# facebookresearch/ProcedureVRL

Measured on AMD Instinct MI355X. Metric: training clips/sec (8f x 224^2, ViT-B TimeSformer), higher is better.
Workload: dtype f16; 1 GPU; TimeSformer ViT-B 8x224^2, 32 clips/GPU, K=9871 step logits, top-5 KL + all-gather InfoNCE, fwd+bwd+AdamW (BASELINE configs[1]; configs[2] at 8 GPUs); clips_per_gpu=32, global_batch=32, parallelism=dp1

## Files before the change

include/pvrl.h:

```cpp
#ifndef PVRL_H_
#define PVRL_H_
#include <stdint.h>
#ifdef __cplusplus
extern "C" {
#endif

#define PVRL_EPI_BF16 0
#define PVRL_EPI_GELU 1
#define PVRL_EPI_QGELU 2
#define PVRL_EPI_RESID_F32 3
#define PVRL_EPI_F32 4
#define PVRL_EPI_DGELU 5
#define PVRL_EPI_DQGELU 6
#define PVRL_EPI_RESID_16 7
#define PVRL_EPI_GELU_ONLY 8

int pvrl_operand_dtype(void);

#define PVRL_NT_SKINNY_MAX_M 192
#define PVRL_NT_SKINNY_K 256
int pvrl_gemm_nt_bf16(const void* A, int64_t lda, const void* W, int64_t ldw, int64_t M, int64_t N, int64_t K,
                      int epilogue, const float* bias, const float* rowscale, const void* aux, int64_t aux_ld,
                      int64_t aux_rowmod, void* out0, int64_t ld0, void* out1, int64_t ld1, const float* bias2,
                      void* stream);

typedef struct pvrl_nt_problem {
  const void* A; int64_t lda;
  const void* W; int64_t ldw;
  int64_t M, N, K;
  const float* bias;
  const float* rowscale;
  const void* aux; int64_t aux_ld;
  void* out0; int64_t ld0;
} pvrl_nt_problem;
int pvrl_gemm_nt_batched_bf16(int nprob, const pvrl_nt_problem* problems, int epilogue, void* stream);

int64_t pvrl_gemm_nt_f32_small_workspace_bytes(int64_t M, int64_t N, int64_t K);
int pvrl_gemm_nt_f32_small(const float* A, int64_t lda, const float* B, int64_t ldb, const float* bias, float alpha,
                           float* C, int64_t ldc, int64_t M, int64_t N, int64_t K, void* workspace,
                           int64_t workspace_bytes, void* stream);

int64_t pvrl_gemm_tn_plan_splits(int64_t M, int64_t N, int64_t K);
int64_t pvrl_gemm_tn_workspace_bytes(int64_t N, int64_t K, int64_t splits);
int pvrl_gemm_tn_bf16(const void* P, int64_t ldp, const void* Q, int64_t ldq, int64_t M, int64_t N, int64_t K,
                      int64_t splits, float beta, float* dW, float* dbias, void* workspace, int64_t workspace_bytes,
                      const float* gscale, float* nonfinite, void* stream);
int pvrl_gemm_tn_into_bf16(const void* P, int64_t ldp, const void* Q, int64_t ldq, int64_t M, int64_t N, int64_t K,
                           int64_t splits, float beta, float* dW, int64_t ldw, int64_t n_valid, int64_t k_valid,
// ... 268 lines not shown
```

procedurevrl_amd/csrc/common.h:

```cpp
#pragma once
#include <hip/hip_runtime.h>
#include <stdint.h>
#include <stdlib.h>

#if defined(PVRL_OPERAND_F16)
typedef _Float16 op_t;
#define PVRL_OPERAND_CODE 1
#define MFMA_16x16x32 __builtin_amdgcn_mfma_f32_16x16x32_f16
#define MFMA_32x32x16 __builtin_amdgcn_mfma_f32_32x32x16_f16
#define FDOT2_F32 __builtin_amdgcn_fdot2
#else
typedef __bf16 op_t;
#define PVRL_OPERAND_CODE 0
#define MFMA_16x16x32 __builtin_amdgcn_mfma_f32_16x16x32_bf16
#define MFMA_32x32x16 __builtin_amdgcn_mfma_f32_32x32x16_bf16
#define FDOT2_F32 __builtin_amdgcn_fdot2_f32_bf16
#endif
typedef op_t opx2 __attribute__((ext_vector_type(2)));
typedef op_t opx4 __attribute__((ext_vector_type(4)));
typedef op_t opx8 __attribute__((ext_vector_type(8)));
typedef short s16x4 __attribute__((ext_vector_type(4)));
typedef float f32x2 __attribute__((ext_vector_type(2)));
typedef float f32x4 __attribute__((ext_vector_type(4)));
typedef float f32x16 __attribute__((ext_vector_type(16)));
// ... 51 lines not shown
#pragma unroll
  for (int o = 32; o > 0; o >>= 1) v = fmaxf(v, __shfl_xor(v, o, 64));
  return v;
}

__device__ __forceinline__ float gelu_clamp6(float u) {
  const float a = fabsf(u);
  return a > 6.0f ? 6.0f : a;
}
__device__ __forceinline__ float gelu_erf(float u) {
  const float x = gelu_clamp6(u);
  float p = fmaf(-2.9932052711956203e-05f, x, 0.0007281892467290163f);
  p = fmaf(p, x, -0.007909782230854034f);
  p = fmaf(p, x, 0.053108397871255875f);
  p = fmaf(p, x, 0.45901164412498474f);
  p = fmaf(p, x, 1.1511247158050537f);
  p = fmaf(p, x, 1.0f);
  const float h = __builtin_amdgcn_exp2f(-p);
  return fmaf(-x, h, fmaxf(u, 0.0f));
}
typedef float f32x2_t __attribute__((ext_vector_type(2)));
__device__ __forceinline__ f32x2_t gelu_erf2(f32x2_t u) {
  const f32x2_t x = {gelu_clamp6(u[0]), gelu_clamp6(u[1])};
  f32x2_t p = __builtin_elementwise_fma((f32x2_t)(-2.9932052711956203e-05f), x, (f32x2_t)(0.0007281892467290163f));
  p = __builtin_elementwise_fma(p, x, (f32x2_t)(-0.007909782230854034f));
  p = __builtin_elementwise_fma(p, x, (f32x2_t)(0.053108397871255875f));
  p = __builtin_elementwise_fma(p, x, (f32x2_t)(0.45901164412498474f));
  p = __builtin_elementwise_fma(p, x, (f32x2_t)(1.1511247158050537f));
  p = __builtin_elementwise_fma(p, x, (f32x2_t)(1.0f));
  const f32x2_t h = {__builtin_amdgcn_exp2f(-p[0]), __builtin_amdgcn_exp2f(-p[1])};
  const f32x2_t r = {fmaxf(u[0], 0.0f), fmaxf(u[1], 0.0f)};
  return __builtin_elementwise_fma(-x, h, r);
}
__device__ __forceinline__ float gelu_erf_grad(float u) {
  const float x = gelu_clamp6(u);
  const float e = __builtin_amdgcn_exp2f(x * x * -0.72134752044448170368f);
  float n = fmaf(1.678248281677952e-06f, x, -3.60403792001307e-05f);
  n = fmaf(n, x, 0.00034598674392327666f);
  n = fmaf(n, x, -0.002000307897105813f);
  n = fmaf(n, x, 0.008002669550478458f);
  n = fmaf(n, x, -0.024410134181380272f);
  n = fmaf(n, x, 0.061244383454322815f);
  n = fmaf(n, x, -0.13256259262561798f);
  n = fmaf(n, x, 0.24993102252483368f);
  n = fmaf(n, x, -0.7978806495666504f);
  n = fmaf(n, x, 0.5f);
  return 0.5f + copysignf(0.5f - e * n, u);
}
__device__ __forceinline__ float quick_gelu(float u) {
  return u * __builtin_amdgcn_rcpf(1.0f + __expf(-1.702f * u));
}
__device__ __forceinline__ float quick_gelu_grad(float u) {
  const float s = __builtin_amdgcn_rcpf(1.0f + __expf(-1.702f * u));
  return s * (1.0f + 1.702f * u * (1.0f - s));
}

__device__ __forceinline__ int xcd_remap(int bid, int nwg) {
  const int q = nwg >> 3, r = nwg & 7;
  const int xcd = bid & 7, idx = bid >> 3;
  const int base = (xcd < r) ? xcd * (q + 1) : r * (q + 1) + (xcd - r) * q;
  return base + idx;
}

static inline int cdiv(long a, long b) { return (int)((a + b - 1) / b); }

static inline int pvrl_compute_cus_per_xcd() {
// ... 13 lines not shown
```

procedurevrl_amd/csrc/gemm_nt.hip:

```cpp
#include "gemm_nt_core.h"
#include "gemm_nt8_core.h"
#include "gemm_nt_skinny.h"

bool pvrl_cls_gemm_f32(const float* A, int64_t lda, const float* B, int64_t ldb, const float* bias, float alpha, float* C, int64_t ldc,
                       int64_t M, int64_t N, int64_t K, hipStream_t s, int* status);

namespace {

constexpr int SG_T = 64, SG_K = 32, SG_LD = 68;
__global__ __launch_bounds__(256) void gemm_f32_small_kernel(const float* __restrict__ A, long lda,
                                                             const float* __restrict__ B, long ldb,
                                                             const float* __restrict__ bias, float alpha,
                                                             float* __restrict__ C, long ldc, int M, int N, int K,
                                                             int kchunk, float* __restrict__ part) {
  __shared__ __attribute__((aligned(16))) float sa[SG_K][SG_LD];
  __shared__ __attribute__((aligned(16))) float sb[SG_K][SG_LD];
  const int tid = threadIdx.x;
  const int n0 = blockIdx.x * SG_T, m0 = blockIdx.y * SG_T;
  const int kbeg = blockIdx.z * kchunk, kend = min(K, kbeg + kchunk);
  const int tx = tid & 15, ty = tid >> 4;
  const int lrow = tid >> 2, lk = (tid & 3) * 8;
  float acc[4][4];
#pragma unroll
  for (int i = 0; i < 4; ++i)
// ... 44 lines not shown
  }
}

__global__ __launch_bounds__(256) void f32_small_reduce_kernel(const float* __restrict__ part, int splits, long MN, int N,
                                                               const float* __restrict__ bias, float alpha,
                                                               float* __restrict__ C, long ldc) {
  for (long i = (long)blockIdx.x * 256 + threadIdx.x; i < MN; i += (long)gridDim.x * 256) {
    float a = 0.f;
    for (int z = 0; z < splits; ++z) a += part[(long)z * MN + i];
    const long m = i / N;
    const int n = (int)(i - m * N);
    C[m * ldc + n] = alpha * a + (bias ? bias[n] : 0.f);
  }
}

static int f32_small_plan(int64_t M, int64_t N, int64_t K, int* kchunk_out) {
  const int tiles = cdiv(N, SG_T) * cdiv(M, SG_T);
  int splits = 1;
  if (tiles < 128 && K >= 512) {
    splits = 256 / tiles;
    const int maxs = (int)(K / 128);
    if (splits > maxs) splits = maxs;
    if (splits < 1) splits = 1;
  }
  const int kchunk = cdiv(cdiv(K, splits), SG_K) * SG_K;
  if (kchunk_out) *kchunk_out = kchunk;
  return cdiv(K, kchunk);
}

constexpr int NT_MID_M = 2048;

template <int EPI>
int launch_nt(const GemmNT& p, hipStream_t s) {
  constexpr bool act_out = EPI == PVRL_EPI_GELU || EPI == PVRL_EPI_QGELU || EPI == PVRL_EPI_GELU_ONLY;
  if (nt_skinny_ok(p)) return launch_nt_skinny<EPI>(p, s);
  if (p.N == 768 && p.M >= 4096 && p.M < 20000) return launch_tile<EPI, 2, 6>(p, s);
  if (p.M >= 4096 && p.N % 256 == 0) {
    if (p.K >= 2 * BK && !(EPI == PVRL_EPI_RESID_16 && p.aux_rowmod != 0)) return launch_nt8<EPI>(p, s);
    return launch_tile<EPI, 4, 4>(p, s);
  }
  if (p.M >= 4096 && p.N % 256 != 0) {
    if (p.N % 384 == 0 && p.M >= 100000) return launch_tile<EPI, 2, 6>(p, s);
    if (p.N % 320 == 0) return launch_tile<EPI, 2, 5>(p, s);
  }
  if (p.M >= NT_MID_M && (p.N % 256 == 0 || act_out)) return launch_tile<EPI, 4, 2>(p, s);
  return launch_tile<EPI, 2, 2>(p, s);
}

}

extern "C" int pvrl_gemm_nt_bf16(const void* A, int64_t lda, const void* W, int64_t ldw, int64_t M, int64_t N,
                                 int64_t K, int epilogue, const float* bias, const float* rowscale,
                                 const void* aux, int64_t aux_ld, int64_t aux_rowmod, void* out0, int64_t ld0,
                                 void* out1, int64_t ld1, const float* bias2, void* stream) {
  if (M <= 0) return PVRL_OK;
  if (bias2 && epilogue != PVRL_EPI_RESID_F32 && epilogue != PVRL_EPI_RESID_16) return PVRL_EINVAL;
  if (!A || !W || !out0 || N <= 0 || K <= 0 || (N % 128) || (K % BK)) return PVRL_EINVAL;
  if ((lda % 8) || (ldw % 8) || (ld0 % 8)) return PVRL_EINVAL;
  if ((epilogue == PVRL_EPI_GELU || epilogue == PVRL_EPI_QGELU) && (!out1 || (ld1 % 8))) return PVRL_EINVAL;
  if ((epilogue == PVRL_EPI_RESID_F32 || epilogue == PVRL_EPI_RESID_16 || epilogue == PVRL_EPI_DGELU || epilogue == PVRL_EPI_DQGELU) &&
      (!aux || (aux_ld % 8)))
    return PVRL_EINVAL;
  GemmNT p;
  p.A = (const op_t*)A; p.lda = lda; p.W = (const op_t*)W; p.ldw = ldw;
  p.M = (int)M; p.N = (int)N; p.K = (int)K;
  p.bias = bias; p.bias2 = bias2; p.rowscale = rowscale; p.aux = aux; p.aux_ld = aux_ld; p.aux_rowmod = (int)aux_rowmod;
  p.out0 = out0; p.ld0 = ld0; p.out1 = out1; p.ld1 = ld1; p.m_off = 0; p.gm = 0;
  p.cus = pvrl_compute_cus_per_xcd(); p.tails = 1;
  hipStream_t s = (hipStream_t)stream;
  switch (epilogue) {
    case PVRL_EPI_BF16: return launch_nt<PVRL_EPI_BF16>(p, s);
    case PVRL_EPI_GELU: return launch_nt<PVRL_EPI_GELU>(p, s);
    case PVRL_EPI_QGELU: return launch_nt<PVRL_EPI_QGELU>(p, s);
    case PVRL_EPI_RESID_F32: return launch_nt<PVRL_EPI_RESID_F32>(p, s);
    case PVRL_EPI_F32: return launch_nt<PVRL_EPI_F32>(p, s);
    case PVRL_EPI_DGELU: return launch_nt<PVRL_EPI_DGELU>(p, s);
    case PVRL_EPI_DQGELU: return launch_nt<PVRL_EPI_DQGELU>(p, s);
    case PVRL_EPI_RESID_16: return launch_nt<PVRL_EPI_RESID_16>(p, s);
    case PVRL_EPI_GELU_ONLY: return launch_nt<PVRL_EPI_GELU_ONLY>(p, s);
    default: return PVRL_EINVAL;
  }
}

extern "C" int pvrl_gemm_nt_batched_bf16(int nprob, const pvrl_nt_problem* problems, int epilogue, void* stream) {
  if (nprob <= 0) return PVRL_OK;
  if (!problems || (epilogue != PVRL_EPI_BF16 && epilogue != PVRL_EPI_F32 && epilogue != PVRL_EPI_RESID_F32)) return PVRL_EINVAL;
  hipStream_t s = (hipStream_t)stream;
  for (int i0 = 0; i0 < nprob; i0 += NT_BATCH_MAX) {
    GemmNTBatch g = {};
    g.n = nprob - i0 < NT_BATCH_MAX ? nprob - i0 : NT_BATCH_MAX;
    int blocks = 0;
    for (int i = 0; i < g.n; ++i) {
      const pvrl_nt_problem& q = problems[i0 + i];
      if (!q.A || !q.W || !q.out0 || q.M <= 0 || q.N <= 0 || q.K <= 0 || (q.N % 128) || (q.K % BK)) return PVRL_EINVAL;
      if ((q.lda % 8) || (q.ldw % 8) || (q.ld0 % 8) || (epilogue == PVRL_EPI_RESID_F32 && (!q.aux || (q.aux_ld % 8)))) return PVRL_EINVAL;
      GemmNT& p = g.prob[i];
      p.A = (const op_t*)q.A; p.lda = q.lda; p.W = (const op_t*)q.W; p.ldw = q.ldw;
      p.M = (int)q.M; p.N = (int)q.N; p.K = (int)q.K;
      p.bias = q.bias; p.bias2 = nullptr; p.rowscale = q.rowscale; p.aux = q.aux; p.aux_ld = q.aux_ld; p.aux_rowmod = 0;
      p.out0 = q.out0; p.ld0 = q.ld0; p.out1 = nullptr; p.ld1 = 0; p.m_off = 0;
      p.cus = pvrl_compute_cus_per_xcd(); p.tails = 0;
      p.tiles_n = p.N / 128; p.tiles_m = cdiv(p.M, 128); p.gm = NT_GM;
      p.nwg = 8 * cdiv(p.tiles_m, 8) * p.tiles_n;
      g.first[i] = blocks;
      blocks += p.nwg;
    }
    g.first[g.n] = blocks;
    switch (epilogue) {
      case PVRL_EPI_BF16: hipLaunchKernelGGL(gemm_nt_batched_kernel<PVRL_EPI_BF16>, dim3(blocks), dim3(256), 0, s, g); break;
      case PVRL_EPI_F32: hipLaunchKernelGGL(gemm_nt_batched_kernel<PVRL_EPI_F32>, dim3(blocks), dim3(256), 0, s, g); break;
      default: hipLaunchKernelGGL(gemm_nt_batched_kernel<PVRL_EPI_RESID_F32>, dim3(blocks), dim3(256), 0, s, g); break;
    }
// ... 34 lines not shown
```

procedurevrl_amd/csrc/gemm_nt8_core.h:

```cpp
#pragma once
#include "gemm_nt_core.h"

namespace {

constexpr int NT8_HALF = 128 * BK * 2;
constexpr int NT8_BUF = 4 * NT8_HALF;

struct Nt8Plan { int full, L, nblk; };
__host__ __device__ inline Nt8Plan nt8_plan(int cm, int tiles_n, int cus, int enable) {
  Nt8Plan t;
  const int T = cm * tiles_n;
  t.full = T;
  t.L = 0;
  if (enable) {
    const int full = (T / cus) * cus, L = T - full;
    if (L > 0 && 2 * L <= cus) { t.full = full; t.L = L; }
  }
  t.nblk = t.full + 2 * t.L;
  return t;
}

#pragma clang diagnostic push
#pragma clang diagnostic ignored "-Winline-asm"
__device__ __forceinline__ void bdma16(rsrc_t r, unsigned voff, unsigned soff, unsigned lds) {
  asm volatile("s_nop 4\n\ts_mov_b32 m0, %3\n\ts_nop 0\n\tbuffer_load_dwordx4 %0, %1, %2 offen lds"
               :: "v"(voff), "s"(r), "s"(soff), "s"(lds) : "memory", "m0");
}
#pragma clang diagnostic pop

template <int EPI>
constexpr int NT8_EB = EPI == PVRL_EPI_RESID_F32 ? 2 : 4;

#define NT8_BARRIER()                       \
  do {                                      \
    __builtin_amdgcn_sched_barrier(0);      \
    __builtin_amdgcn_s_barrier();           \
    __builtin_amdgcn_sched_barrier(0);      \
  } while (0)
#define NT8_MEM_END()                                     \
  do {                                                    \
    asm volatile("s_waitcnt lgkmcnt(0)" ::: "memory");    \
    NT8_BARRIER();                                        \
    __builtin_amdgcn_s_setprio(1);                        \
  } while (0)
#define NT8_CMP_END()                 \
  do {                                \
    __builtin_amdgcn_s_setprio(0);    \
    NT8_BARRIER();                    \
  } while (0)

template <int EPI>
__global__ __launch_bounds__(512, 2) void gemm_nt8_kernel(GemmNT p) {
  constexpr bool F32OUT = (EPI == PVRL_EPI_RESID_F32 || EPI == PVRL_EPI_F32);
  constexpr int EB = NT8_EB<EPI>;
  constexpr int NST = (F32OUT || EPI == PVRL_EPI_GELU || EPI == PVRL_EPI_QGELU) ? 32 : 16;
  __shared__ __attribute__((aligned(16))) char smem[2 * NT8_BUF];
  const int tid = threadIdx.x, lane = tid & 63;
  const int wave = __builtin_amdgcn_readfirstlane(tid >> 6);
  const int wm = wave >> 2, wn = wave & 3;
  const unsigned sbase = __builtin_amdgcn_readfirstlane(lds_addr(smem));
  const int nk = p.K / BK;

  const int xcd = blockIdx.x & 7, stride = gridDim.x >> 3;
  const int qm = p.tiles_m >> 3, rm = p.tiles_m & 7;
  const int cm = qm + (xcd < rm ? 1 : 0);
  const int mbase = xcd * qm + (xcd < rm ? xcd : rm);
  const Nt8Plan plan = nt8_plan(cm, p.tiles_n, p.cus, p.tails);
  const int GM = p.gm, gsz = GM * p.tiles_n;
  auto decode = [&](int e, int& tm, int& tn) {
    const int g = e / gsz, r = e - g * gsz;
    const int gm = min(GM, cm - g * GM);
    tn = r / gm;
    tm = mbase + g * GM + (r - tn * gm);
    tn = __builtin_amdgcn_readfirstlane(tn);
    tm = __builtin_amdgcn_readfirstlane(tm);
  };
  int j = blockIdx.x >> 3;
  if (j >= plan.nblk) return;

  unsigned voffA[2][2], voffW[2];
#pragma unroll
  for (int e = 0; e < 2; ++e) {
    const int row = 16 * wave + 8 * e + (lane >> 3), pc = lane & 7;
#pragma unroll
    for (int h = 0; h < 2; ++h) voffA[h][e] = (unsigned)(128 * h + row) * (unsigned)p.lda * 2u + ((unsigned)(pc ^ swz_x(row)) << 4);
    voffW[e] = (unsigned)row * (unsigned)p.ldw * 2u + ((unsigned)(pc ^ swz_w<F32OUT>(row)) << 4);
  }
  const unsigned wstep = 128u * (unsigned)p.ldw * 2u;
// ... 203 lines not shown
```

procedurevrl_amd/csrc/gemm_nt_core.h:

```cpp
#pragma once
#include <algorithm>
#include "common.h"
#include "../../include/pvrl.h"

namespace {

struct GemmNT {
  const op_t* A; long lda;
  const op_t* W; long ldw;
  int M, N, K;
  const float* bias;
  const float* bias2;
  const float* rowscale;
  const void* aux;
  long aux_ld; int aux_rowmod;
  void* out0; long ld0;
  void* out1; long ld1;
  int tiles_m, tiles_n, nwg;
  int cus, tails;
  int m_off;
  int gm;
};

constexpr int BK = 64;
constexpr int NT_GM = 6;

__device__ __forceinline__ int swz_x(int row) { return (row >> 1) & 7; }
template <bool F32OUT> __device__ __forceinline__ int w_row(int nt, int i) {
  return 32 * (nt >> 1) + 8 * (i >> 2) + 4 * (nt & 1) + (i & 3);
}
template <bool F32OUT> __device__ __forceinline__ int swz_w(int row) {
  return ((row >> 1) & 1) | (((row >> 3) & 3) << 1);
}

typedef __amdgpu_buffer_rsrc_t rsrc_t;
__device__ __forceinline__ rsrc_t tile_rsrc(const void* base, long row0, long ld, int elem, int rows) {
  return __builtin_amdgcn_make_buffer_rsrc((void*)((const char*)base + row0 * ld * elem), 0, (int)(rows * ld * elem), 0x00020000);
}
__device__ __forceinline__ void bst16(rsrc_t r, unsigned off, f32x4 v) {
  __builtin_amdgcn_raw_buffer_store_b128(__builtin_bit_cast(u32x4, v), r, off, 0, 0);
}
__device__ __forceinline__ void bst16(rsrc_t r, unsigned off, opx8 v) {
  __builtin_amdgcn_raw_buffer_store_b128(__builtin_bit_cast(u32x4, v), r, off, 0, 0);
}
template <typename T> __device__ __forceinline__ T bld16(rsrc_t r, unsigned off) {
  return __builtin_bit_cast(T, __builtin_amdgcn_raw_buffer_load_b128(r, off, 0, 0));
}

template <int EPI, int BATCH = 2, bool TAB = false>
__device__ __forceinline__ void nt_epilogue_at(const GemmNT& p, f32x4 (&acc)[4][4], int m0, int n0, int rb, int c0, int c1, int lane) {
  constexpr bool F32OUT = (EPI == PVRL_EPI_RESID_F32 || EPI == PVRL_EPI_F32);
  static_assert(BATCH == 1 || BATCH == 2 || BATCH == 4, "row tiles per load batch");
  const int q = lane >> 4, i = lane & 15;
  const int ncol[2] = {n0 + c0 + 8 * q, n0 + c1 + 8 * q};
  const int rows = __builtin_amdgcn_readfirstlane(max(0, min(1024, p.M - m0)));
  if constexpr (F32OUT) {
    f32x4 bv[4];
#pragma unroll
    for (int nt = 0; nt < 4; ++nt)
      bv[nt] = !p.bias ? (f32x4){0.f, 0.f, 0.f, 0.f} : *reinterpret_cast<const f32x4*>(p.bias + ncol[nt >> 1] + 4 * (nt & 1));
    float rs4[4];
#pragma unroll
    for (int mt = 0; mt < 4; ++mt) rs4[mt] = p.rowscale ? p.rowscale[min(m0 + rb + mt * 16 + i, p.M - 1)] : 1.f;
    float b2lane = 0.f;
    if constexpr (EPI == PVRL_EPI_RESID_F32) {
      if (p.bias2) {
        b2lane = p.bias2[n0 + (lane < 32 ? c0 + lane : c1 + lane - 32)];
        if (!p.rowscale) {
#pragma unroll
          for (int nt = 0; nt < 4; ++nt)
#pragma unroll
            for (int e = 0; e < 4; ++e) bv[nt][e] += __shfl(b2lane, 32 * (nt >> 1) + 8 * q + 4 * (nt & 1) + e, 64);
        }
      }
    }
    const bool b2_late = EPI == PVRL_EPI_RESID_F32 && p.bias2 && p.rowscale;
    const rsrc_t ro = tile_rsrc(p.out0, m0, p.ld0, 4, rows);
    const bool tab = EPI == PVRL_EPI_RESID_F32 && p.aux_rowmod != 0;
    const rsrc_t ra = EPI == PVRL_EPI_RESID_F32 ? (tab ? tile_rsrc(p.aux, 0, p.aux_ld, 4, p.aux_rowmod) : tile_rsrc(p.aux, m0, p.aux_ld, 4, rows)) : ro;
#pragma unroll
    for (int bt = 0; bt < 4 / BATCH; ++bt) {
// ... 29 lines not shown
            }
          }
          bst16(ro, ob + (unsigned)(ncol[nt >> 1] + 4 * (nt & 1)) * 4u, ov);
        }
      }
    }
  } else {
    float bv[2][8];
#pragma unroll
    for (int c = 0; c < 2; ++c)
#pragma unroll
      for (int e = 0; e < 8; ++e) bv[c][e] = !p.bias ? 0.f : p.bias[ncol[c] + e];
    float rs4[4];
#pragma unroll
    for (int mt = 0; mt < 4; ++mt) rs4[mt] = p.rowscale ? p.rowscale[min(m0 + rb + mt * 16 + i, p.M - 1)] : 1.f;
    constexpr bool TWO = EPI == PVRL_EPI_GELU || EPI == PVRL_EPI_QGELU;
    constexpr bool DACT = EPI == PVRL_EPI_DGELU || EPI == PVRL_EPI_DQGELU;
    constexpr bool RES16 = EPI == PVRL_EPI_RESID_16;
    constexpr bool tab = RES16 && TAB;
    float b2lane = 0.f;
    if constexpr (RES16) {
      if (p.bias2) {
        b2lane = p.bias2[n0 + (lane < 32 ? c0 + lane : c1 + lane - 32)];
        if (!p.rowscale) {
#pragma unroll
          for (int c = 0; c < 2; ++c)
#pragma unroll
            for (int e = 0; e < 8; ++e) bv[c][e] += __shfl(b2lane, 32 * c + 8 * q + e, 64);
        }
      }
    }
    const bool b2_late = RES16 && p.bias2 && p.rowscale;
    const rsrc_t r0 = tile_rsrc(p.out0, m0, p.ld0, 2, rows);
    const rsrc_t r1 = TWO ? tile_rsrc(p.out1, m0, p.ld1, 2, rows) : r0;
    const rsrc_t ra = (DACT || RES16) ? (tab ? tile_rsrc(p.aux, 0, p.aux_ld, 4, p.aux_rowmod) : tile_rsrc(p.aux, m0, p.aux_ld, 2, rows)) : r0;
#pragma unroll
    for (int bt = 0; bt < 4 / BATCH; ++bt) {
      opx8 uv[BATCH][2];
      if constexpr ((DACT || RES16) && !tab) {
#pragma unroll
        for (int h = 0; h < BATCH; ++h) {
          const unsigned ab = (unsigned)(rb + (BATCH * bt + h) * 16 + i) * (unsigned)p.aux_ld * 2u;
#pragma unroll
          for (int c = 0; c < 2; ++c) uv[h][c] = bld16<opx8>(ra, ab + (unsigned)ncol[c] * 2u);
        }
      }
#pragma unroll
      for (int h = 0; h < BATCH; ++h) {
        const int mt = BATCH * bt + h;
        const unsigned ml = (unsigned)(rb + mt * 16 + i);
        const float rs = rs4[mt];
#pragma unroll
        for (int c = 0; c < 2; ++c) {
          float v[8];
#pragma unroll
          for (int e = 0; e < 4; ++e) {
            v[e] = acc[mt][2 * c][e] + bv[c][e];
            v[4 + e] = acc[mt][2 * c + 1][e] + bv[c][4 + e];
          }
          const unsigned o0off = ml * (unsigned)p.ld0 * 2u + (unsigned)ncol[c] * 2u;
          if constexpr (EPI == PVRL_EPI_BF16) {
            opx8 o0;
#pragma unroll
            for (int e = 0; e < 8; ++e) o0[e] = (op_t)(rs * v[e]);
            bst16(r0, o0off, o0);
          } else if constexpr (EPI == PVRL_EPI_GELU_ONLY) {
            opx8 g0;
#pragma unroll
            for (int e = 0; e < 8; e += 2) {
              const f32x2_t gg = gelu_erf2((f32x2_t){v[e], v[e + 1]});
              g0[e] = (op_t)gg[0];
              g0[e + 1] = (op_t)gg[1];
            }
            bst16(r0, o0off, g0);
          } else if constexpr (TWO) {
            opx8 u0, g0;
#pragma unroll
            for (int e = 0; e < 8; e += 2) {
              u0[e] = (op_t)v[e];
              u0[e + 1] = (op_t)v[e + 1];
              if constexpr (EPI == PVRL_EPI_GELU) {
                const f32x2_t gg = gelu_erf2((f32x2_t){v[e], v[e + 1]});
                g0[e] = (op_t)gg[0];
                g0[e + 1] = (op_t)gg[1];
              } else {
                g0[e] = (op_t)quick_gelu(v[e]);
                g0[e + 1] = (op_t)quick_gelu(v[e + 1]);
              }
            }
            bst16(r0, o0off, u0);
            bst16(r1, ml * (unsigned)p.ld1 * 2u + (unsigned)ncol[c] * 2u, g0);
          } else if constexpr (RES16) {
            float a[8];
            if constexpr (tab) {
              const int mr = (min(m0 + (int)ml, p.M - 1) + p.m_off) % p.aux_rowmod;
              const unsigned ab = (unsigned)mr * (unsigned)p.aux_ld * 4u + (unsigned)ncol[c] * 4u;
              const f32x4 t0 = bld16<f32x4>(ra, ab), t1 = bld16<f32x4>(ra, ab + 16u);
#pragma unroll
              for (int e = 0; e < 4; ++e) { a[e] = t0[e]; a[4 + e] = t1[e]; }
            } else {
              const opx8 ua = uv[h][c];
#pragma unroll
              for (int e = 0; e < 8; ++e) a[e] = (float)ua[e];
            }
            if (b2_late) {
#pragma unroll
              for (int e = 0; e < 8; ++e) a[e] += __shfl(b2lane, 32 * c + 8 * q + e, 64);
// ... 250 lines not shown
```

procedurevrl_amd/csrc/gemm_nt_skinny.h:

```cpp
#pragma once
#include "gemm_nt_core.h"

namespace {

constexpr int SK_MT = 3;
constexpr int SK_NW = 8;
constexpr int SK_MAX_M = PVRL_NT_SKINNY_MAX_M;
static_assert(32 * SK_NW == PVRL_NT_SKINNY_K, "include/pvrl.h states the rule the callers read");

template <int EPI>
__global__ __launch_bounds__(64 * SK_NW) void gemm_nt_skinny_kernel(GemmNT p) {
  __shared__ float part[SK_NW][SK_MT][4][64];
  const int tid = threadIdx.x, lane = tid & 63;
  const int wave = __builtin_amdgcn_readfirstlane(tid >> 6);
  const int r = lane & 15, q = lane >> 4;
  const int n0 = blockIdx.x * 16, m0 = blockIdx.y * (16 * SK_MT);
  const int mt_n = min(SK_MT, (p.M - m0 + 15) >> 4);
  const int kw = p.K / SK_NW, kbeg = wave * kw;
  const op_t* wrow = p.W + (long)(n0 + r) * p.ldw + kbeg + q * 8;
  const op_t* xrow[SK_MT];
#pragma unroll
  for (int t = 0; t < SK_MT; ++t) xrow[t] = p.A + (long)min(m0 + t * 16 + r, p.M - 1) * p.lda + kbeg + q * 8;
  f32x4 acc[SK_MT];
#pragma unroll
// ... 24 lines not shown
    if constexpr (EPI == PVRL_EPI_RESID_F32) {
      if (p.bias2 && !p.rowscale) b += p.bias2[n];
      const long ar = p.aux_rowmod ? (long)((m + p.m_off) % p.aux_rowmod) : (long)m;
      float v = rs * (s + b) + reinterpret_cast<const float*>(p.aux)[ar * p.aux_ld + n];
      if (p.bias2 && p.rowscale) v += p.bias2[n];
      reinterpret_cast<float*>(p.out0)[(long)m * p.ld0 + n] = v;
    } else if constexpr (EPI == PVRL_EPI_RESID_16) {
      if (p.bias2 && !p.rowscale) b += p.bias2[n];
      const float a = p.aux_rowmod ? reinterpret_cast<const float*>(p.aux)[(long)((m + p.m_off) % p.aux_rowmod) * p.aux_ld + n]
                                   : (float)reinterpret_cast<const op_t*>(p.aux)[(long)m * p.aux_ld + n];
      float v = rs * (s + b) + a;
      if (p.bias2 && p.rowscale) v += p.bias2[n];
      reinterpret_cast<op_t*>(p.out0)[(long)m * p.ld0 + n] = (op_t)v;
    } else if constexpr (EPI == PVRL_EPI_F32) {
      reinterpret_cast<float*>(p.out0)[(long)m * p.ld0 + n] = rs * (s + b);
    } else if constexpr (EPI == PVRL_EPI_BF16) {
      reinterpret_cast<op_t*>(p.out0)[(long)m * p.ld0 + n] = (op_t)(rs * (s + b));
    } else if constexpr (EPI == PVRL_EPI_GELU_ONLY) {
      const float u = s + b;
      reinterpret_cast<op_t*>(p.out0)[(long)m * p.ld0 + n] = (op_t)gelu_erf2((f32x2_t){u, u})[0];
    } else if constexpr (EPI == PVRL_EPI_GELU || EPI == PVRL_EPI_QGELU) {
      const float u = s + b;
      reinterpret_cast<op_t*>(p.out0)[(long)m * p.ld0 + n] = (op_t)u;
      reinterpret_cast<op_t*>(p.out1)[(long)m * p.ld1 + n] =
          (op_t)(EPI == PVRL_EPI_GELU ? gelu_erf2((f32x2_t){u, u})[0] : quick_gelu(u));
    } else {
      const float ua = (float)reinterpret_cast<const op_t*>(p.aux)[(long)m * p.aux_ld + n];
      const float d = EPI == PVRL_EPI_DGELU ? gelu_erf_grad(ua) : quick_gelu_grad(ua);
      reinterpret_cast<op_t*>(p.out0)[(long)m * p.ld0 + n] = (op_t)(rs * (s + b) * d);
    }
  }
}

inline bool nt_skinny_ok(const GemmNT& p) { return p.M <= SK_MAX_M && p.K % (32 * SK_NW) == 0 && p.N % 16 == 0; }

template <int EPI>
int launch_nt_skinny(const GemmNT& p, hipStream_t s) {
  hipLaunchKernelGGL((gemm_nt_skinny_kernel<EPI>), dim3((unsigned)(p.N / 16), (unsigned)cdiv(p.M, 16 * SK_MT)), dim3(64 * SK_NW), 0, s, p);
  PVRL_LAUNCH_CHECK();
  return PVRL_OK;
}

}
```

procedurevrl_amd/engine.py:

```python
import math
import os

import torch

from . import ops
from ._lib import lib
from .grads import SCALED_GRADS, GradStore
from .graphs import GraphReplay, drop_graphs_quietly
from .transform import DecodedClips

OP16 = ops.OP16
F32 = torch.float32


class _X:
    __slots__ = ("p", "c", "full")

    def __init__(self, p, c, full=None):
        self.p, self.c, self.full = p, c, full

    @staticmethod
    def new(R, B, C, device, split, zero=False, zero_p=True):
        mk = torch.zeros if zero else torch.empty
        if split:
# ... 326 lines not shown

    def saved_nbytes(self):
        return storage_nbytes(self.saved)

    def stream_from_rows(self, x_rows, B):
        R = x_rows.shape[0] - B
        if not self.resid16:
            full = x_rows.contiguous()
            return _X(full[:R], full[R:], full)
        return _X(x_rows[:R].to(OP16).contiguous(), x_rows[R:].contiguous())

    @staticmethod
    def stream_to_rows(x):
        return x.full if x.full is not None else torch.cat([x.p.float(), x.c], 0)

    def _undef(self, t):
        if self.debug_nan_undefined and t is not None and t.numel():
            t.fill_(float("nan"))
        return t

    def _epi_resid(self):
        L = lib()
        return L.PVRL_EPI_RESID_16 if self.resid16 else L.PVRL_EPI_RESID_F32

    def _cls_mlp_fp32(self, blk, xc, s3c, out):
        P = lambda t: t.detach()
        hc, _, _ = ops.layernorm_fwd(xc, P(blk.norm2.weight), P(blk.norm2.bias), self.eps, out_dtype=F32, save_stats=False)
        gc = ops.cls_linear(hc, P(blk.mlp.fc1.weight), P(blk.mlp.fc1.bias), gelu=True)
        ops.cls_linear(gc, P(blk.mlp.fc2.weight), P(blk.mlp.fc2.bias), rowscale=s3c, biasscale=s3c, aux=xc, out=out)

    def _fc1(self, blk, h_m, keep_u):
        L = lib()
        w1, b1 = self._weight(blk.mlp.fc1.weight).w, blk.mlp.fc1.bias.detach()
        if keep_u:
            return ops.gemm_nt(h_m, w1, L.PVRL_EPI_GELU, bias=b1)
        return None, ops.gemm_nt(h_m, w1, L.PVRL_EPI_GELU_ONLY, bias=b1)

    def _mlp_fwd(self, blk, x, s3_all, sv, whole=False, keep_u=True, recompute=False):
        L = lib()
        B, R = sv["B"], sv["R"]
        P = lambda t: t.detach()
        h_m, mean_m, rstd_m = ops.layernorm_fwd(x.all(), P(blk.norm2.weight), P(blk.norm2.bias), self.eps)
        u, g = self._fc1(blk, h_m, keep_u)
        if recompute:
            return None, h_m, (mean_m, rstd_m), u, g
        y = _X.new(R, B, self.C, x.c.device, sv["split"])
        s3c = s3_all[R:] if s3_all is not None else None
        w2 = self._weight(blk.mlp.fc2.weight).w
        if whole:
            ops.gemm_nt(g, w2, L.PVRL_EPI_RESID_F32, bias=P(blk.mlp.fc2.bias), rowscale=s3_all, aux=x.full, out0=y.full)
        else:
            ops.gemm_nt(g[:R], w2, self._epi_resid(), bias=P(blk.mlp.fc2.bias), rowscale=s3_all[:R] if s3_all is not None else None,
                        aux=x.p, out0=y.p)
            if not self.cls_fp32:
                ops.gemm_nt(g[R:], w2, L.PVRL_EPI_RESID_F32, bias=P(blk.mlp.fc2.bias), rowscale=s3c, aux=x.c, out0=y.c)
        if self.cls_fp32:
            self._cls_mlp_fp32(blk, x.c, s3c, y.c)
        return y, h_m, (mean_m, rstd_m), u, g

    def _mlp_bwd(self, blk, s, dy, gs):
        L = lib()
        self._lin_wgrad(gs, dy, s["g"], blk.mlp.fc2)
        du = ops.gemm_nt(dy, self._weight(blk.mlp.fc2.weight).t, L.PVRL_EPI_DGELU, aux=s["u"])
        self._lin_wgrad(gs, du, s["h_m"], blk.mlp.fc1)
        return ops.gemm_nt(du, self._weight(blk.mlp.fc1.weight).t, L.PVRL_EPI_BF16)

    def _block_fwd(self, blk, x0, sv, dp, save, last=False, ckpt=False, recompute=False):
        prune = last and self.prune_last
        keep_u = save and not ckpt
        L = lib()
        B, T, N, R, M = sv["B"], sv["T"], sv["N"], sv["R"], sv["M"]
        C, H = self.C, self.H
        dev = x0.c.device
        split, epi_res = sv["split"], self._epi_resid()
        s1_tok = dp["s1_tok"] if dp else None
        s2_seq = dp["s2_seq"] if dp else None
        s2_tok = dp["s2_tok"] if dp else None
        s3_all = dp["s3_all"] if dp else None
        P = lambda t: t.detach()

        h_t, mean_t, rstd_t = ops.layernorm_fwd(x0.patch(), P(blk.temporal_norm1.weight), P(blk.temporal_norm1.bias), self.eps)
        qkv_t = ops.gemm_nt(h_t, self._weight(blk.temporal_attn.qkv.weight).w, L.PVRL_EPI_BF16,
                            bias=P(blk.temporal_attn.qkv.bias))
        lse_t = None
        if T == 8:
            o_t = ops.attn_t8_fwd(qkv_t, B * N, H, self.scale)
        else:
            o_t, _, lse_t = ops.attn_fwd(qkv_t, B * N, T, H, self.scale, mode=0)
        if split:
            x1 = _X(torch.empty_like(x0.p), x0.c)
        else:
            x1 = _X.new(R, B, C, dev, False)
        fe = self._fused_temporal(blk)
        ops.gemm_nt(o_t, fe.w, epi_res, bias=fe.be, rowscale=s1_tok, bias2=P(blk.temporal_fc.bias),
                    aux=x0.p, out0=x1.p)
        if not split:
# ... 231 lines not shown
            G = G * gs.inv
            dcls_rows = dcls_rows * gs.inv
        gs.accumulate(m.cls_token, dcls_rows.view(1, 1, C), fused=True, checks=False)
        dpos = torch.cat([dcls_rows.unsqueeze(0), G.sum(1)], 0)
        dtime = G.sum(0)
        pos_p, tim_p = m.pos_embed, None if self.space_only else m.time_embed
        if pos_p.shape[1] != N + 1 or (tim_p is not None and tim_p.shape[1] != T):
            raise NotImplementedError("training with resized pos/time embeddings is not supported (reference "
                                      "resizes at inference only, vit.py:374)")
        gs.accumulate(pos_p, dpos.unsqueeze(0), fused=True, checks=False)
        if tim_p is not None:
            gs.accumulate(tim_p, dtime.unsqueeze(0), fused=True, checks=False)
        self.flush_wgrads()
        self._finish_deferred(gs)
        if gs.scale is not None:
            gs.end_scaled()
        self.saved = None

    def _block_bwd(self, blk, s, sv, dx, gs, dy, has_prev, prev_dp, dxp_zero=False):
        L = lib()
        B, T, N, R, M = sv["B"], sv["T"], sv["N"], sv["R"], sv["M"]
        C, H = self.C, self.H
        dev = dx.c.device
        if s.get("undivided"):
            return self._block_bwd_undivided(blk, s, sv, dx, gs, dy, has_prev, prev_dp)
        dp = s["dp"]
        s1_tok = dp["s1_tok"] if dp else None
        s2_seq = dp["s2_seq"] if dp else None
        s2_tok = dp["s2_tok"] if dp else None
        s3_all = dp["s3_all"] if dp else None

        if s.get("pruned"):
            wq = [self._lin_wgrad(gs, dy, s["g"], blk.mlp.fc2, queue=False)]
            du = ops.gemm_nt(dy, self._weight(blk.mlp.fc2.weight).t, L.PVRL_EPI_DGELU, aux=s["u"])
            wq.append(self._lin_wgrad(gs, du, s["h_m"], blk.mlp.fc1, queue=False))
            dh = ops.gemm_nt(du, self._weight(blk.mlp.fc1.weight).t, L.PVRL_EPI_BF16)
            self._lnbwd(gs, dh, s["x2"].c, s["st_m"], blk.norm2, dx.c, dx.c)
            dpc = ops.group_bcast(dx.c, B, T, scale=s2_seq, alpha=1.0 / T)
            wq.append(self._lin_wgrad(gs, dpc, s["o_s"][R:], blk.attn.proj, queue=False))
            if not s.get("cls_attn"):
                ops.gemm_tn_grouped(wq, ws_tag="tn_cls")
            if s.get("cls_attn"):
                do = ops.gemm_nt(dpc, self._weight(blk.attn.proj.weight).t, L.PVRL_EPI_BF16)
            else:
                do = torch.zeros((R + B * T, C), device=dev, dtype=OP16)
                ops.gemm_nt(dpc, self._weight(blk.attn.proj.weight).t, L.PVRL_EPI_BF16, out0=do[R:])
            del du, dpc
        else:
            dh = self._mlp_bwd(blk, s, dy, gs)
            dps = torch.empty((R + B * T, C), device=dev, dtype=OP16)
            self._lnbwd(gs, dh, s["x2"].all(), s["st_m"], blk.norm2, dx.all(), dx.all(), dxs=dps[:R], dxs_scale=s2_tok)

            ops.group_bcast(dx.c, B, T, scale=s2_seq, alpha=1.0 / T, out=dps[R:])
            self._lin_wgrad(gs, dps, s["o_s"], blk.attn.proj)
            do = ops.gemm_nt(dps, self._weight(blk.attn.proj.weight).t, L.PVRL_EPI_BF16)
            del dps
        dqkv = torch.empty((M + B * T, 3 * C), device=dev, dtype=OP16)
        if s.get("cls_attn"):
            self._undef(dqkv[:R, :C])
            ops.attn_cls_bwd(s["qkv_s"], s["o_s"][R:], do, s["lse_s"], B * T, N + 1, H, self.scale, T, R, dqkv[:M], dqkv[M:],
                             zero_patch_dq=False)
            ops.group_reduce(dqkv[M:], B, T, out=dqkv[R:M])
            (dw, bw), (dbias, _) = gs.target(blk.attn.qkv.weight, fused=True), gs.target(blk.attn.qkv.bias, fused=True)
            wq.append((dqkv[R:M, :C], s["h_s"][R:], dw[:C], dbias[:C], bw, gs.inv, gs.bad))
            ops.gemm_tn_grouped(wq, ws_tag="tn_cls")
            self._wgrad(dqkv[:M, C:], s["h_s"], dw[C:], dbias[C:], bw, gscale=gs.inv, nonfinite=gs.bad)
            wt = self._weight(blk.attn.qkv.weight).t
# ... 36 lines not shown
```

procedurevrl_amd/ops.py:

```python
import ctypes

import torch

from ._lib import lib, PvrlError, header_constants, operand_torch_dtype

_HC = header_constants()
NT_SKINNY_MAX_M, NT_SKINNY_K, TN_GROUP_MAX = _HC["PVRL_NT_SKINNY_MAX_M"], _HC["PVRL_NT_SKINNY_K"], _HC["PVRL_TN_GROUP_MAX"]
HEAD_DIM = _HC["PVRL_HEAD_DIM"]
OP16 = operand_torch_dtype()
F32 = torch.float32

KERNEL_TIMING = None
_EPI_NAMES = {0: "op16", 1: "gelu", 2: "qgelu", 3: "resid_f32", 4: "f32", 5: "dgelu", 6: "dqgelu", 7: "resid_16", 8: "gelu_only"}


def _timed(name, flops, fn):
    if KERNEL_TIMING is None:
        return fn()
    e0 = torch.cuda.Event(enable_timing=True)
    e1 = torch.cuda.Event(enable_timing=True)
    e0.record()
    r = fn()
    e1.record()
    KERNEL_TIMING.append((name, flops, e0, e1))
    return r


def collect_kernel_timing():
    if not KERNEL_TIMING:
        return None
    torch.cuda.synchronize()
    agg = {}
    for name, flops, e0, e1 in KERNEL_TIMING:
        a = agg.setdefault(name, [0, 0.0, 0.0])
        a[0] += 1
        a[1] += e0.elapsed_time(e1)
        a[2] += flops
    summary = {k: {"calls": v[0], "ms": round(v[1], 3), "avg_us": round(1e3 * v[1] / v[0], 2),
                   "tflops": round(v[2] / (v[1] * 1e-3) / 1e12, 1) if v[1] > 0 else 0.0} for k, v in agg.items()}
    order = sorted(agg.items(), key=lambda kv: -kv[1][1])

    def roof_of(item):
        name, (calls, ms, flops) = item
        ach = flops / (ms * 1e-3) / 1e12
        return {"kernel": name, "bound": "mfma", "achieved": round(ach, 1), "peak": 2500.0, "unit": "TFLOP/s",
                "frac": round(ach / 2500.0, 4), "traffic": None, "calls": calls, "avg_launch_us": round(1e3 * ms / calls, 2),
# ... 18 lines not shown

def _chk2d(t, dtype=None):
    if t.dim() != 2 or (t.stride(1) != 1 and t.shape[1] != 1):
        raise PvrlError(f"expected a row-major 2-D tensor, got shape {tuple(t.shape)} stride {t.stride()}")
    if not t.is_cuda:
        raise PvrlError("the HIP path needs device tensors (no CPU fallback)")
    if dtype is not None and t.dtype != dtype:
        raise PvrlError(f"expected dtype {dtype}, got {t.dtype}")
    return t


def _ld(t):
    return t.stride(0) if t.shape[0] > 1 else max(t.stride(0), t.shape[1])


def _ptr_ld(t):
    return (None, 0) if t is None else (_ptr(t), _ld(t))


def gemm_nt(A, W, epi, bias=None, rowscale=None, aux=None, aux_rowmod=0, out0=None, out1=None, bias2=None):
    L = lib()
    _chk2d(A, OP16); _chk2d(W, OP16)
    M, K = A.shape
    N = W.shape[0]
    assert W.shape[1] == K
    f32_out = epi in (L.PVRL_EPI_RESID_F32, L.PVRL_EPI_F32)
    if out0 is None:
        out0 = torch.empty((M, N), device=A.device, dtype=F32 if f32_out else OP16)
    if out0.dtype != (F32 if f32_out else OP16) or (epi == L.PVRL_EPI_RESID_16 and aux.dtype != (F32 if aux_rowmod else OP16)):
        raise PvrlError(f"gemm_nt epilogue {_EPI_NAMES[epi]}: out0 {out0.dtype}, aux {None if aux is None else aux.dtype}")
    two = epi in (L.PVRL_EPI_GELU, L.PVRL_EPI_QGELU)
    if two and out1 is None:
        out1 = torch.empty((M, N), device=A.device, dtype=OP16)
    fam = "gemm_nt_skinny<" if (M <= NT_SKINNY_MAX_M and K % NT_SKINNY_K == 0) else "gemm_nt_kernel<"
    _timed(fam + _EPI_NAMES[epi] + ">", 2.0 * M * N * K, lambda: L.call(
        "pvrl_gemm_nt_bf16", _ptr(A), _ld(A), _ptr(W), _ld(W), M, N, K, epi, _ptr(bias), _ptr(rowscale),
        *_ptr_ld(aux), aux_rowmod, _ptr(out0), _ld(out0),
        *_ptr_ld(out1), _ptr(bias2), _stream()))
    return (out0, out1) if two else out0


def gemm_nt_batched(problems, epi):
    from ._lib import NtProblem
    L = lib()
    if not problems:
        return []
    f32_out = epi in (L.PVRL_EPI_RESID_F32, L.PVRL_EPI_F32)
    arr = (NtProblem * len(problems))()
    outs, flops = [], 0.0
    for a, pr in zip(arr, problems):
        A, W = _chk2d(pr["A"], OP16), _chk2d(pr["W"], OP16)
        M, K = A.shape
        N = W.shape[0]
        assert W.shape[1] == K
        out0 = pr.get("out0")
        if out0 is None:
            out0 = torch.empty((M, N), device=A.device, dtype=F32 if f32_out else OP16)
        aux, bias, rs = pr.get("aux"), pr.get("bias"), pr.get("rowscale")
        a.A, a.lda, a.W, a.ldw, a.M, a.N, a.K = A.data_ptr(), _ld(A), W.data_ptr(), _ld(W), M, N, K
        a.bias = None if bias is None else bias.data_ptr()
        a.rowscale = None if rs is None else rs.data_ptr()
        a.aux, a.aux_ld = _ptr_ld(aux)
        a.out0, a.ld0 = out0.data_ptr(), _ld(out0)
        outs.append(out0)
        flops += 2.0 * M * N * K
    _timed("gemm_nt_batched<" + _EPI_NAMES[epi] + ">", flops, lambda: L.call(
        "pvrl_gemm_nt_batched_bf16", len(problems), ctypes.addressof(arr), epi, _stream()))
    return outs


def gemm_nt_f32(A, B, bias=None, alpha=1.0, out=None):
    L = lib()
# ... 736 lines not shown
```

Before: 733.8 clips/s.

## Store quantized 12-bit GELU derivative codes instead of fc1 pre-activations

The fc1 GEMM epilogue now computes the GELU derivative alongside the activation and stores it as a packed 12-bit code (1.5 bytes per element) in place of the 16-bit pre-activation. The fc2 backward dgrad epilogue unpacks these codes and multiplies by them directly, so the backward pass no longer recomputes the erf-based derivative. This cuts saved-activation memory and bandwidth for the MLP hidden state and removes transcendental work from the backward. In exchange the GELU gradient is quantized to about 3e-4 resolution, which may affect training numerics, and the few-row skinny kernel path is not available for these epilogues.

```diff
diff --git a/include/pvrl.h b/include/pvrl.h
--- a/include/pvrl.h
+++ b/include/pvrl.h
@@ -14,6 +14,8 @@
 #define PVRL_EPI_DQGELU 6
 #define PVRL_EPI_RESID_16 7
 #define PVRL_EPI_GELU_ONLY 8
+#define PVRL_EPI_GELU_C12 9
+#define PVRL_EPI_DGELU_C12 10
 
 int pvrl_operand_dtype(void);
 
diff --git a/procedurevrl_amd/csrc/common.h b/procedurevrl_amd/csrc/common.h
--- a/procedurevrl_amd/csrc/common.h
+++ b/procedurevrl_amd/csrc/common.h
@@ -107,6 +107,21 @@
   const f32x2_t r = {fmaxf(u[0], 0.0f), fmaxf(u[1], 0.0f)};
   return __builtin_elementwise_fma(-x, h, r);
 }
+__device__ __forceinline__ f32x2_t gelu_erf2_G(f32x2_t u, f32x2_t& G) {
+  const f32x2_t x = {gelu_clamp6(u[0]), gelu_clamp6(u[1])};
+  f32x2_t p = __builtin_elementwise_fma((f32x2_t)(-2.9932052711956203e-05f), x, (f32x2_t)(0.0007281892467290163f));
+  p = __builtin_elementwise_fma(p, x, (f32x2_t)(-0.007909782230854034f));
+  p = __builtin_elementwise_fma(p, x, (f32x2_t)(0.053108397871255875f));
+  p = __builtin_elementwise_fma(p, x, (f32x2_t)(0.45901164412498474f));
+  p = __builtin_elementwise_fma(p, x, (f32x2_t)(1.1511247158050537f));
+  p = __builtin_elementwise_fma(p, x, (f32x2_t)(1.0f));
+  const f32x2_t h = {__builtin_amdgcn_exp2f(-p[0]), __builtin_amdgcn_exp2f(-p[1])};
+  const f32x2_t r = {fmaxf(u[0], 0.0f), fmaxf(u[1], 0.0f)};
+  const f32x2_t xx = x * x * (f32x2_t)(-0.72134752044448170368f);
+  const f32x2_t e = {__builtin_amdgcn_exp2f(xx[0]), __builtin_amdgcn_exp2f(xx[1])};
+  G = __builtin_elementwise_fma(x * (f32x2_t)(-0.3989422804014327f), e, h);
+  return __builtin_elementwise_fma(-x, h, r);
+}
 __device__ __forceinline__ float gelu_erf_grad(float u) {
   const float x = gelu_clamp6(u);
   const float e = __builtin_amdgcn_exp2f(x * x * -0.72134752044448170368f);
diff --git a/procedurevrl_amd/csrc/gemm_nt.hip b/procedurevrl_amd/csrc/gemm_nt.hip
--- a/procedurevrl_amd/csrc/gemm_nt.hip
+++ b/procedurevrl_amd/csrc/gemm_nt.hip
@@ -100,8 +100,10 @@
 
 template <int EPI>
 int launch_nt(const GemmNT& p, hipStream_t s) {
-  constexpr bool act_out = EPI == PVRL_EPI_GELU || EPI == PVRL_EPI_QGELU || EPI == PVRL_EPI_GELU_ONLY;
-  if (nt_skinny_ok(p)) return launch_nt_skinny<EPI>(p, s);
+  constexpr bool act_out = EPI == PVRL_EPI_GELU || EPI == PVRL_EPI_QGELU || EPI == PVRL_EPI_GELU_ONLY || EPI == PVRL_EPI_GELU_C12;
+  if constexpr (NT_SKINNY_EPI<EPI>) {
+    if (nt_skinny_ok<EPI>(p)) return launch_nt_skinny<EPI>(p, s);
+  }
   if (p.N == 768 && p.M >= 4096 && p.M < 20000) return launch_tile<EPI, 2, 6>(p, s);
   if (p.M >= 4096 && p.N % 256 == 0) {
     if (p.K >= 2 * BK && !(EPI == PVRL_EPI_RESID_16 && p.aux_rowmod != 0)) return launch_nt8<EPI>(p, s);
@@ -129,6 +131,8 @@
   if ((epilogue == PVRL_EPI_RESID_F32 || epilogue == PVRL_EPI_RESID_16 || epilogue == PVRL_EPI_DGELU || epilogue == PVRL_EPI_DQGELU) &&
       (!aux || (aux_ld % 8)))
     return PVRL_EINVAL;
+  if (epilogue == PVRL_EPI_GELU_C12 && (!out1 || (ld1 % 8) || ld1 < N)) return PVRL_EINVAL;
+  if (epilogue == PVRL_EPI_DGELU_C12 && (!aux || (aux_ld % 8) || aux_ld < N)) return PVRL_EINVAL;
   GemmNT p;
   p.A = (const op_t*)A; p.lda = lda; p.W = (const op_t*)W; p.ldw = ldw;
   p.M = (int)M; p.N = (int)N; p.K = (int)K;
@@ -146,6 +150,8 @@
     case PVRL_EPI_DQGELU: return launch_nt<PVRL_EPI_DQGELU>(p, s);
     case PVRL_EPI_RESID_16: return launch_nt<PVRL_EPI_RESID_16>(p, s);
     case PVRL_EPI_GELU_ONLY: return launch_nt<PVRL_EPI_GELU_ONLY>(p, s);
+    case PVRL_EPI_GELU_C12: return launch_nt<PVRL_EPI_GELU_C12>(p, s);
+    case PVRL_EPI_DGELU_C12: return launch_nt<PVRL_EPI_DGELU_C12>(p, s);
     default: return PVRL_EINVAL;
   }
 }
diff --git a/procedurevrl_amd/csrc/gemm_nt8_core.h b/procedurevrl_amd/csrc/gemm_nt8_core.h
--- a/procedurevrl_amd/csrc/gemm_nt8_core.h
+++ b/procedurevrl_amd/csrc/gemm_nt8_core.h
@@ -53,7 +53,7 @@
 __global__ __launch_bounds__(512, 2) void gemm_nt8_kernel(GemmNT p) {
   constexpr bool F32OUT = (EPI == PVRL_EPI_RESID_F32 || EPI == PVRL_EPI_F32);
   constexpr int EB = NT8_EB<EPI>;
-  constexpr int NST = (F32OUT || EPI == PVRL_EPI_GELU || EPI == PVRL_EPI_QGELU) ? 32 : 16;
+  constexpr int NST = (F32OUT || EPI == PVRL_EPI_GELU || EPI == PVRL_EPI_QGELU || EPI == PVRL_EPI_GELU_C12) ? 32 : 16;
   __shared__ __attribute__((aligned(16))) char smem[2 * NT8_BUF];
   const int tid = threadIdx.x, lane = tid & 63;
   const int wave = __builtin_amdgcn_readfirstlane(tid >> 6);
diff --git a/procedurevrl_amd/csrc/gemm_nt_core.h b/procedurevrl_amd/csrc/gemm_nt_core.h
--- a/procedurevrl_amd/csrc/gemm_nt_core.h
+++ b/procedurevrl_amd/csrc/gemm_nt_core.h
@@ -47,6 +47,27 @@
   return __builtin_bit_cast(T, __builtin_amdgcn_raw_buffer_load_b128(r, off, 0, 0));
 }
 
+typedef unsigned u32x3 __attribute__((ext_vector_type(3)));
+constexpr float C12_LO = 0.13f, C12_Q = 1.26f / 4095.0f, C12_RQ = 4095.0f / 1.26f;
+__device__ __forceinline__ unsigned c12_code(float G, float v) {
+  const float t = copysignf(fmaf(G, -C12_RQ, 0.5f * C12_RQ), v) + ((0.5f + C12_LO) * C12_RQ + 0.5f);
+  return min((unsigned)t, 4095u);
+}
+__device__ __forceinline__ u32x3 c12_pack(const unsigned (&c)[8]) {
+  return (u32x3){c[0] | (c[1] << 12) | (c[2] << 24), (c[2] >> 8) | (c[3] << 4) | (c[4] << 16) | (c[5] << 28),
+                 (c[5] >> 4) | (c[6] << 8) | (c[7] << 20)};
+}
+__device__ __forceinline__ void c12_unpack(u32x3 w, float (&d)[8]) {
+  const unsigned w01 = __builtin_amdgcn_alignbit(w[1], w[0], 24), w12 = __builtin_amdgcn_alignbit(w[2], w[1], 28);
+  const unsigned c[8] = {__builtin_amdgcn_ubfe(w[0], 0, 12), __builtin_amdgcn_ubfe(w[0], 12, 12), __builtin_amdgcn_ubfe(w01, 0, 12),
+                         __builtin_amdgcn_ubfe(w[1], 4, 12), __builtin_amdgcn_ubfe(w[1], 16, 12), __builtin_amdgcn_ubfe(w12, 0, 12),
+                         __builtin_amdgcn_ubfe(w[2], 8, 12), w[2] >> 20};
+#pragma unroll
+  for (int e = 0; e < 8; ++e) d[e] = fmaf((float)c[e], C12_Q, -C12_LO);
+}
+__device__ __forceinline__ void bst12(rsrc_t r, unsigned off, u32x3 v) { __builtin_amdgcn_raw_buffer_store_b96(v, r, off, 0, 0); }
+__device__ __forceinline__ u32x3 bld12(rsrc_t r, unsigned off) { return __builtin_amdgcn_raw_buffer_load_b96(r, off, 0, 0); }
+
 template <int EPI, int BATCH = 2, bool TAB = false>
 __device__ __forceinline__ void nt_epilogue_at(const GemmNT& p, f32x4 (&acc)[4][4], int m0, int n0, int rb, int c0, int c1, int lane) {
   constexpr bool F32OUT = (EPI == PVRL_EPI_RESID_F32 || EPI == PVRL_EPI_F32);
@@ -142,8 +163,11 @@
     }
     const bool b2_late = RES16 && p.bias2 && p.rowscale;
     const rsrc_t r0 = tile_rsrc(p.out0, m0, p.ld0, 2, rows);
-    const rsrc_t r1 = TWO ? tile_rsrc(p.out1, m0, p.ld1, 2, rows) : r0;
-    const rsrc_t ra = (DACT || RES16) ? (tab ? tile_rsrc(p.aux, 0, p.aux_ld, 4, p.aux_rowmod) : tile_rsrc(p.aux, m0, p.aux_ld, 2, rows)) : r0;
+    constexpr bool C12F = EPI == PVRL_EPI_GELU_C12, C12B = EPI == PVRL_EPI_DGELU_C12;
+    const unsigned cpitch = (unsigned)((C12F ? p.ld1 : p.aux_ld) * 3 / 2);
+    const rsrc_t r1 = TWO ? tile_rsrc(p.out1, m0, p.ld1, 2, rows) : C12F ? tile_rsrc(p.out1, m0, cpitch, 1, rows) : r0;
+    const rsrc_t ra = (DACT || RES16) ? (tab ? tile_rsrc(p.aux, 0, p.aux_ld, 4, p.aux_rowmod) : tile_rsrc(p.aux, m0, p.aux_ld, 2, rows))
+                      : C12B ? tile_rsrc(p.aux, m0, cpitch, 1, rows) : r0;
 #pragma unroll
     for (int bt = 0; bt < 4 / BATCH; ++bt) {
       opx8 uv[BATCH][2];
@@ -153,6 +177,15 @@
           const unsigned ab = (unsigned)(rb + (BATCH * bt + h) * 16 + i) * (unsigned)p.aux_ld * 2u;
 #pragma unroll
           for (int c = 0; c < 2; ++c) uv[h][c] = bld16<opx8>(ra, ab + (unsigned)ncol[c] * 2u);
+        }
+      }
+      u32x3 cv[BATCH][2];
+      if constexpr (C12B) {
+#pragma unroll
+        for (int h = 0; h < BATCH; ++h) {
+          const unsigned ab = (unsigned)(rb + (BATCH * bt + h) * 16 + i) * cpitch;
+#pragma unroll
+          for (int c = 0; c < 2; ++c) cv[h][c] = bld12(ra, ab + (unsigned)ncol[c] * 3u / 2u);
         }
       }
 #pragma unroll
@@ -183,6 +216,27 @@
               g0[e + 1] = (op_t)gg[1];
             }
             bst16(r0, o0off, g0);
+          } else if constexpr (C12F) {
+            opx8 g0;
+            unsigned cc[8];
+#pragma unroll
+            for (int e = 0; e < 8; e += 2) {
+              f32x2_t G;
+              const f32x2_t gg = gelu_erf2_G((f32x2_t){v[e], v[e + 1]}, G);
+              g0[e] = (op_t)gg[0];
+              g0[e + 1] = (op_t)gg[1];
+              cc[e] = c12_code(G[0], v[e]);
+              cc[e + 1] = c12_code(G[1], v[e + 1]);
+            }
+            bst16(r0, o0off, g0);
+            bst12(r1, ml * cpitch + (unsigned)ncol[c] * 3u / 2u, c12_pack(cc));
+          } else if constexpr (C12B) {
+            float d[8];
+            c12_unpack(cv[h][c], d);
+            opx8 o0;
+#pragma unroll
+            for (int e = 0; e < 8; ++e) o0[e] = (op_t)(rs * v[e] * d[e]);
+            bst16(r0, o0off, o0);
           } else if constexpr (TWO) {
             opx8 u0, g0;
 #pragma unroll
diff --git a/procedurevrl_amd/csrc/gemm_nt_skinny.h b/procedurevrl_amd/csrc/gemm_nt_skinny.h
--- a/procedurevrl_amd/csrc/gemm_nt_skinny.h
+++ b/procedurevrl_amd/csrc/gemm_nt_skinny.h
@@ -80,10 +80,13 @@
   }
 }
 
-inline bool nt_skinny_ok(const GemmNT& p) { return p.M <= SK_MAX_M && p.K % (32 * SK_NW) == 0 && p.N % 16 == 0; }
+template <int EPI> constexpr bool NT_SKINNY_EPI = EPI != PVRL_EPI_GELU_C12 && EPI != PVRL_EPI_DGELU_C12;
+template <int EPI>
+inline bool nt_skinny_ok(const GemmNT& p) { return NT_SKINNY_EPI<EPI> && p.M <= SK_MAX_M && p.K % (32 * SK_NW) == 0 && p.N % 16 == 0; }
 
 template <int EPI>
 int launch_nt_skinny(const GemmNT& p, hipStream_t s) {
+  static_assert(NT_SKINNY_EPI<EPI>, "no few-row kernel for the code epilogues");
   hipLaunchKernelGGL((gemm_nt_skinny_kernel<EPI>), dim3((unsigned)(p.N / 16), (unsigned)cdiv(p.M, 16 * SK_MT)), dim3(64 * SK_NW), 0, s, p);
   PVRL_LAUNCH_CHECK();
   return PVRL_OK;
diff --git a/procedurevrl_amd/engine.py b/procedurevrl_amd/engine.py
--- a/procedurevrl_amd/engine.py
+++ b/procedurevrl_amd/engine.py
@@ -382,8 +382,10 @@
     def _fc1(self, blk, h_m, keep_u):
         L = lib()
         w1, b1 = self._weight(blk.mlp.fc1.weight).w, blk.mlp.fc1.bias.detach()
-        if keep_u:
-            return ops.gemm_nt(h_m, w1, L.PVRL_EPI_GELU, bias=b1)
+        few_rows = h_m.shape[0] <= ops.NT_SKINNY_MAX_M and h_m.shape[1] % ops.NT_SKINNY_K == 0
+        if keep_u or few_rows:
+            code, g = ops.gemm_nt(h_m, w1, L.PVRL_EPI_GELU_C12, bias=b1)
+            return (code if keep_u else None), g
         return None, ops.gemm_nt(h_m, w1, L.PVRL_EPI_GELU_ONLY, bias=b1)
 
     def _mlp_fwd(self, blk, x, s3_all, sv, whole=False, keep_u=True, recompute=False):
@@ -411,7 +413,7 @@
     def _mlp_bwd(self, blk, s, dy, gs):
         L = lib()
         self._lin_wgrad(gs, dy, s["g"], blk.mlp.fc2)
-        du = ops.gemm_nt(dy, self._weight(blk.mlp.fc2.weight).t, L.PVRL_EPI_DGELU, aux=s["u"])
+        du = ops.gemm_nt(dy, self._weight(blk.mlp.fc2.weight).t, L.PVRL_EPI_DGELU_C12, aux=s["u"])
         self._lin_wgrad(gs, du, s["h_m"], blk.mlp.fc1)
         return ops.gemm_nt(du, self._weight(blk.mlp.fc1.weight).t, L.PVRL_EPI_BF16)
 
@@ -709,7 +711,7 @@
 
         if s.get("pruned"):
             wq = [self._lin_wgrad(gs, dy, s["g"], blk.mlp.fc2, queue=False)]
-            du = ops.gemm_nt(dy, self._weight(blk.mlp.fc2.weight).t, L.PVRL_EPI_DGELU, aux=s["u"])
+            du = ops.gemm_nt(dy, self._weight(blk.mlp.fc2.weight).t, L.PVRL_EPI_DGELU_C12, aux=s["u"])
             wq.append(self._lin_wgrad(gs, du, s["h_m"], blk.mlp.fc1, queue=False))
             dh = ops.gemm_nt(du, self._weight(blk.mlp.fc1.weight).t, L.PVRL_EPI_BF16)
             self._lnbwd(gs, dh, s["x2"].c, s["st_m"], blk.norm2, dx.c, dx.c)
diff --git a/procedurevrl_amd/ops.py b/procedurevrl_amd/ops.py
--- a/procedurevrl_amd/ops.py
+++ b/procedurevrl_amd/ops.py
@@ -11,7 +11,8 @@
 F32 = torch.float32
 
 KERNEL_TIMING = None
-_EPI_NAMES = {0: "op16", 1: "gelu", 2: "qgelu", 3: "resid_f32", 4: "f32", 5: "dgelu", 6: "dqgelu", 7: "resid_16", 8: "gelu_only"}
+_EPI_NAMES = {0: "op16", 1: "gelu", 2: "qgelu", 3: "resid_f32", 4: "f32", 5: "dgelu", 6: "dqgelu", 7: "resid_16", 8: "gelu_only",
+              9: "gelu_c12", 10: "dgelu_c12"}
 
 
 def _timed(name, flops, fn):
@@ -96,12 +97,39 @@
     two = epi in (L.PVRL_EPI_GELU, L.PVRL_EPI_QGELU)
     if two and out1 is None:
         out1 = torch.empty((M, N), device=A.device, dtype=OP16)
+    if epi in (L.PVRL_EPI_GELU_C12, L.PVRL_EPI_DGELU_C12):
+        return _gemm_nt_c12(L, A, W, epi, bias, rowscale, aux, out0, out1)
     fam = "gemm_nt_skinny<" if (M <= NT_SKINNY_MAX_M and K % NT_SKINNY_K == 0) else "gemm_nt_kernel<"
     _timed(fam + _EPI_NAMES[epi] + ">", 2.0 * M * N * K, lambda: L.call(
         "pvrl_gemm_nt_bf16", _ptr(A), _ld(A), _ptr(W), _ld(W), M, N, K, epi, _ptr(bias), _ptr(rowscale),
         *_ptr_ld(aux), aux_rowmod, _ptr(out0), _ld(out0),
         *_ptr_ld(out1), _ptr(bias2), _stream()))
     return (out0, out1) if two else out0
+
+
+def _code_ld(code, N):
+    _chk2d(code, torch.uint8)
+    pitch = _ld(code)
+    if code.shape[1] != N * 3 // 2 or pitch % 12:
+        raise PvrlError(f"code matrix of {N} columns: expected uint8 [M, {N * 3 // 2}] with a pitch of whole 12-byte groups, got "
+                        f"{tuple(code.shape)} stride {code.stride()}")
+    return pitch * 2 // 3
+
+
+def _gemm_nt_c12(L, A, W, epi, bias, rowscale, code_in, out0, code_out):
+    (M, K), N = A.shape, W.shape[0]
+    fwd = epi == L.PVRL_EPI_GELU_C12
+    if fwd and code_out is None:
+        code_out = torch.empty((M, N * 3 // 2), device=A.device, dtype=torch.uint8)
+    code = code_out if fwd else code_in
+    if code is None or code.shape[0] != M:
+        raise PvrlError(f"gemm_nt epilogue {_EPI_NAMES[epi]}: needs the [M, N * 3 // 2] uint8 code matrix")
+    ld = _code_ld(code, N)
+    _timed("gemm_nt_kernel<" + _EPI_NAMES[epi] + ">", 2.0 * M * N * K, lambda: L.call(
+        "pvrl_gemm_nt_bf16", _ptr(A), _ld(A), _ptr(W), _ld(W), M, N, K, epi, _ptr(bias), _ptr(rowscale),
+        None if fwd else _ptr(code), 0 if fwd else ld, 0, _ptr(out0), _ld(out0),
+        _ptr(code) if fwd else None, ld if fwd else 0, None, _stream()))
+    return (code, out0) if fwd else out0
 
 
 def gemm_nt_batched(problems, epi):
```

Result: no change. 739.0 clips/s (median of 6 runs) (+0.7%).
